# samholt/NeuralLaplaceControl

Hardware: AMD Instinct MI355X
Metric: MPPI planning steps/sec (16384 samples, H=40) (higher is better)
Workload: dtype f64

## Files before the change

### neurallaplacecontrol_amd/csrc/abi_ctx.hip

```cpp
#include "nlc_host.h"

using namespace nlc;
using namespace nlc::host;

namespace nlc {
namespace host {

thread_local std::string g_create_error;

bool gru_use_coop(const nlc_ctx* c, int64_t n_windows) {
  if (c->opt.gru_coop >= 0) return c->opt.gru_coop != 0;
  if (c->g == 128) return true;
  return n_windows <= (c->g == 32 ? 8192 : 50000);
}

void prof_flush(nlc_ctx* c) {
  for (auto& p : c->prof) {
    for (auto& ev : p.pending) {
      hipEventSynchronize(ev.second);
      float ms = 0.f;
      hipEventElapsedTime(&ms, ev.first, ev.second);
      p.total_ms += ms;
      c->event_pool.push_back(ev.first);
      c->event_pool.push_back(ev.second);
// ... 74 lines not shown
    return NLC_OK;
  } catch (...) {
    g_create_error = "exception in nlc_create";
    return NLC_ERR_STATE;
  }
}

extern "C" void nlc_destroy(nlc_ctx* c) {
  if (!c) return;
  hipSetDevice(c->device);
  hipStreamSynchronize(c->stream);
  nlc_comm_destroy(c);
  prof_flush(c);
  if (c->arena.base) hipFree(c->arena.base);
  if (c->dbg_scratch) hipFree(c->dbg_scratch);
  if (c->rnn_base) hipFree(c->rnn_base);
  if (c->node_base) hipFree(c->node_base);
  if (c->slot_dev) hipFree(c->slot_dev);
  if (c->eidx_dev) hipFree(c->eidx_dev);
  if (c->lin_tab) hipFree(c->lin_tab);
  for (int i = 0; i < 2; ++i)
    if (c->U[i]) hipFree(c->U[i]);
  if (c->b1fold) hipFree(c->b1fold);
  if (c->cp_lin) hipFree(c->cp_lin);
  if (c->b1fold_fwd) hipFree(c->b1fold_fwd);
  if (c->small) hipFree(c->small);
  if (c->pinned) hipHostFree(c->pinned);
  c->dh.destroy();
  c->side.destroy();
  for (hipEvent_t e : c->event_pool) hipEventDestroy(e);
// ... 67 lines not shown
  } else if (n == "fused_roll_cap") {
    if (value < 0) return fail(c, NLC_ERR_BAD_ARG, "fused_roll_cap must be >= 0 (0 = auto)");
    c->opt.fused.roll_cap = (int)value;
  } else if (n == "fused_chain_first_tiles") {
    if (value < -1 || value > 64) return fail(c, NLC_ERR_BAD_ARG, "fused_chain_first_tiles must be in -1..64 (-1 = auto)");
    c->opt.fused.chain_first_tiles = (int)value;
  } else if (n == "fused_partner_tiles") {
    if (value < -2 || value > 64) return fail(c, NLC_ERR_BAD_ARG, "fused_partner_tiles must be in -2..64 (-2 = auto, -1 = never)");
    c->opt.fused.partner_tiles = (int)value;
  } else if (n == "repfunc_split") {
    if (value != 0 && value != 1) return fail(c, NLC_ERR_BAD_ARG, "repfunc_split must be 0 or 1");
    c->opt.repfunc_split = (int)value;
  } else if (n == "gru_coop") {
    if (value != 0 && value != 1 && value != -1) return fail(c, NLC_ERR_BAD_ARG, "gru_coop must be -1 (auto), 0 or 1");
    c->opt.gru_coop = (int)value;
  } else if (n == "gru_gemm") {
    if (value != 0 && value != 1) return fail(c, NLC_ERR_BAD_ARG, "gru_gemm must be 0 (FP64 MFMA) or 1 (int8-sliced)");
    c->opt.gru_gemm = (int)value;
    if (c->has_model) c->gru.use_i8 = (c->gru.i8_stream != nullptr && value == 1) ? 1 : 0;
  } else if (n == "dbg_gap_us") {
    if (value < 0 || value > 1.0e5) return fail(c, NLC_ERR_BAD_ARG, "dbg_gap_us must be in 0 .. 1e5");
    c->opt.dbg_gap_us = value;
  } else if (n == "dbg_l2_mb") {
    if (value < 0 || value > 4096) return fail(c, NLC_ERR_BAD_ARG, "dbg_l2_mb must be in 0 .. 4096");
    c->opt.dbg_l2_mb = value;
  } else if (n == "fused_max_samples") {
    if (value < 0) return fail(c, NLC_ERR_BAD_ARG, "fused_max_samples must be >= 0");
    c->opt.fused_max_samples = (int64_t)value;
  } else {
    return fail(c, NLC_ERR_BAD_ARG, "unknown option: " + n);
// ... 5 lines not shown
  if (!c) return NLC_ERR_BAD_ARG;
  if (!name || !out) return fail(c, NLC_ERR_BAD_ARG, "NULL stat name / out");
  const std::string n(name);
  if (n == "rollout_body") *out = (double)c->last_body;
  else if (n == "fused_timeouts") *out = (double)c->fused.timeouts;
  else if (n == "fused_fallbacks") *out = (double)c->fused.fallbacks;
  else if (n == "fused_lost") *out = c->fused.lost ? 1.0 : 0.0;
  else if (n == "last_giveup_command") *out = (double)c->fused.last_giveup_command;
  else if (n == "commands") *out = (double)c->commands;
  else if (n == "comm_world") *out = c->comm ? (double)c->comm_world : 0.0;
  else if (n == "comm_rank") *out = c->comm ? (double)c->comm_rank : -1.0;
  else if (n == "fused_blocks_per_cu") *out = (double)c->fused.blocks_per_cu;
  else if (n == "fused_spin_limit") *out = (double)c->opt.fused_spin_limit;
  else if (n == "model_nt3") *out = c->has_model ? (double)c->net.nt3 : 0.0;
  else if (n == "gru_gemm") *out = (c->has_model && c->gru.use_i8) ? 1.0 : 0.0;
  else if (n == "gru_i8_launches") *out = (double)nlc::gru_i8_launch_count();
  else return fail(c, NLC_ERR_BAD_ARG, "unknown stat: " + n);
  return NLC_OK;
}

extern "C" int nlc_synchronize(nlc_ctx* c) {
  if (!c) return NLC_ERR_BAD_ARG;
  NLC_HIP(c, hipStreamSynchronize(c->stream));
  return NLC_OK;
}

extern "C" int nlc_device_info(nlc_ctx* c, char* name, int name_len, int* cus, int* mhz, double* gib) {
  if (!c) return NLC_ERR_BAD_ARG;
  if (name && name_len > 0) {
    std::snprintf(name, name_len, "%s (%s)", c->prop.name, c->prop.gcnArchName);
// ... 34 lines not shown
```

### neurallaplacecontrol_amd/csrc/abi_model.hip

```cpp
#include "nlc_host.h"

using namespace nlc;
using namespace nlc::host;

namespace {
int64_t blob_size(const nlc_model_desc* d) {
  const int64_t g = d->h / 2, S = d->ilt.terms, P = d->d + 2, h = d->h;
  return 3 * g * d->nin + 3 * g * g + 6 * g + 3 * g * g + 3 * g * g + 6 * g + 2 * g + 2 + h * (2 * S + P) + h +
         h * h + h + 2 * d->d * S * h + 2 * d->d * S;
}
}

extern "C" int64_t nlc_model_blob_size(const nlc_model_desc* d) { return d ? blob_size(d) : -1; }

extern "C" int nlc_set_model(nlc_ctx* c, const nlc_model_desc* d, const double* w, int64_t n) {
  if (!c) return NLC_ERR_BAD_ARG;
  NLC_GUARD_BEGIN
  if (!d || !w) return fail(c, NLC_ERR_BAD_ARG, "NULL desc or weights");
  if (int r = check_ilt(c, &d->ilt)) return r;
  if (d->h != 64 && d->h != 128 && d->h != 256)
    return fail(c, NLC_ERR_UNSUPPORTED, "hidden_units must be 64, 128 or 256 (the kernels are instantiated for these widths)");
  if (d->d < 1 || d->d > 6) return fail(c, NLC_ERR_UNSUPPORTED, "state_dim must be in 1..6");
  if (d->nin < 1 || d->nin > NLC_MAX_NIN) return fail(c, NLC_ERR_UNSUPPORTED, "GRU input dim must be in 1..3");
  const bool linear_algo = d->ilt.algo == NLC_ILT_FIXED_TALBOT || d->ilt.algo == NLC_ILT_STEHFEST;
// ... 55 lines not shown
  const size_t o_W1p = ar.push(pack_A(W1p.data(), 8, 8, rowsh));
  const size_t o_b1 = ar.push(std::vector<double>(b1, b1 + h));
  const size_t o_W2 = ar.push(pack_A(W2, h, h, rowsh));
  const size_t o_b2 = ar.push(std::vector<double>(b2, b2 + h));
  const int nt3 = nl_pick_nt3(ilt_tiles_needed(dd, S));
  if (nt3 < 0) return fail(c, NLC_ERR_UNSUPPORTED, "2*d*S too large for the fused kernel (max 25 output tiles)");
  const IltSlots slots = make_ilt_slots(dd, S, nt3);
  c->slot_elems = slots.elems;
  const int n_even_groups = slots.n_even_groups;
  std::vector<double> b3p((size_t)nt3 * 16, 0.0);
  for (size_t i = 0; i < slots.rowmap3.size(); ++i)
    if (slots.rowmap3[i] >= 0) b3p[i] = b3[slots.rowmap3[i]];
  const size_t o_W3 = ar.push(pack_A(W3, h, h, slots.rowmap3));
  const size_t o_b3 = ar.push(b3p);
  const size_t o_Cp = ar.push(slots.Cp);

  double* base = nullptr;
  NLC_HIP(c, hipMalloc((void**)&base, ar.host.size() * sizeof(double)));
  hipError_t e = hipMemcpy(base, ar.host.data(), ar.host.size() * sizeof(double), hipMemcpyHostToDevice);
  if (e != hipSuccess) {
    hipFree(base);
    return fail(c, NLC_ERR_HIP, std::string("weight upload: ") + hipGetErrorString(e));
  }
  {
    std::vector<int> slot((size_t)nt3 * 8, -1);
    for (size_t i = 0; i < slot.size(); ++i)
      if (slots.elems[i].first >= 0) slot[i] = slots.elems[i].first * S + slots.elems[i].second;
    if (c->slot_dev) hipFree(c->slot_dev);
    c->slot_dev = nullptr;
    NLC_HIP(c, hipMalloc((void**)&c->slot_dev, slot.size() * sizeof(int)));
// ... 49 lines not shown
  N.W1s = base + o_W1s;
  N.b1 = base + o_b1;
  N.W2p = base + o_W2;
  N.b2 = base + o_b2;
  N.W3p = base + o_W3;
  N.b3p = base + o_b3;
  N.Cp = base + o_Cp;
  for (int i = 0; i < NLC_MAX_D; ++i) {
    N.state_mean[i] = i < dd ? d->state_mean[i] : 0.0;
    N.state_std[i] = i < dd ? d->state_std[i] : 1.0;
  }
  N.alpha = d->ilt.alpha;
  N.log_tol = std::log(d->ilt.tol);
  N.scale = d->ilt.scale;
  N.time_div = d->time_div;
  c->has_model = true;
  c->fwd_tn = -1.0;
  c->has_mppi = false;
  return NLC_OK;
  NLC_GUARD_END(c)
}

extern "C" int nlc_gru_encode(nlc_ctx* c, const double* window, int64_t N, int B, double* out) {
  if (!c) return NLC_ERR_BAD_ARG;
  NLC_GUARD_BEGIN
  if (!c->has_model) return fail(c, NLC_ERR_STATE, "nlc_set_model has not been called");
  if (N < 0 || B < 1) return fail(c, NLC_ERR_BAD_SHAPE, "bad N or B");
  if (N == 0) return NLC_OK;
  if (!window || !out) return fail(c, NLC_ERR_BAD_ARG, "NULL device pointer");
  NLC_HIP(c, hipSetDevice(c->device));
// ... 215 lines not shown
```

### neurallaplacecontrol_amd/csrc/abi_planner.hip

```cpp
#include "nlc_host.h"

using namespace nlc;
using namespace nlc::host;

extern "C" int nlc_mppi_configure(nlc_ctx* c, const nlc_mppi_desc* d) {
  if (!c) return NLC_ERR_BAD_ARG;
  NLC_GUARD_BEGIN
  if (!d) return fail(c, NLC_ERR_BAD_ARG, "NULL desc");
  if (d->K < 1 || d->T < 1 || d->K_global < d->K || d->k_offset < 0 || d->k_offset + d->K > d->K_global)
    return fail(c, NLC_ERR_BAD_SHAPE, "bad K / K_global / k_offset / T");
  if (d->nu < 1 || d->nu > NLC_MAX_NU) return fail(c, NLC_ERR_UNSUPPORTED, "nu must be 1 or 2");
  if (d->d < 1 || (d->d > NLC_MAX_D && d->dynamics != NLC_DYN_EXTERNAL)) return fail(c, NLC_ERR_BAD_SHAPE, "bad nx");
  if (d->B < 1) return fail(c, NLC_ERR_BAD_SHAPE, "action_buffer needs at least one row");
  if (!(d->lambda_ > 0.0) || d->u_scale == 0.0) return fail(c, NLC_ERR_BAD_ARG, "lambda_ must be > 0, u_scale != 0");
  if (d->u_per_command < 1 || d->u_per_command > d->T) return fail(c, NLC_ERR_BAD_ARG, "bad u_per_command");
  if (d->E < 0 || d->E > 65535) return fail(c, NLC_ERR_BAD_ARG, "episodes E must be in [0, 65535]");
  const int E = d->E < 1 ? 1 : d->E;
  if ((double)E * (double)d->K * d->T * d->nu > 2.0e9)
    return fail(c, NLC_ERR_BAD_SHAPE, "E*K*T*nu exceeds the planner's index range");
  const bool env_free = d->cost_external &&
                        (d->dynamics == NLC_DYN_NL || d->dynamics == NLC_DYN_DTRNN || d->dynamics == NLC_DYN_NODE) &&
                        d->env == -1;
  if (!env_free && (d->env < 0 || d->env > NLC_ENV_CARTPOLE_NOTRIG)) return fail(c, NLC_ERR_UNSUPPORTED, "unknown env id");
  static const int env_d[4] = {5, 3, 6, 4}, env_nu[4] = {1, 1, 2, 1};
// ... 64 lines not shown
        for (int lane = 0; lane < 64; ++lane) {
          const auto el = c->slot_elems[(size_t)4 * g + (lane >> 4)];
          if (el.first != (lane & 15)) continue;
          cp[(size_t)g * 64 + lane] = tab[2 * S + el.second] / c->tn;
          cp[(size_t)(ng + g) * 64 + lane] = -tab[3 * S + el.second] / c->tn;
        }
      if (c->opt.test_lin_coeff_scale != 1.0) {
        size_t at = 0;
        for (size_t i = 0; i < cp.size(); ++i)
          if (std::fabs(cp[i]) > std::fabs(cp[at])) at = i;
        cp[at] *= c->opt.test_lin_coeff_scale;
      }
      if (int rc = hold_doubles(c, c->cp_lin, cp.size(), cp.data())) return rc;
    }
  }
  c->has_mppi = true;
  c->dh.reset();
  c->wait.reset();
  c->fused.new_problem();
  return NLC_OK;
  NLC_GUARD_END(c)
}

namespace nlc {
namespace host {
bool linear_on_rollout_kernels(const nlc_ctx* c) {
  return c->has_model && (c->md.ilt.algo == NLC_ILT_FIXED_TALBOT || c->md.ilt.algo == NLC_ILT_STEHFEST) &&
         (c->md.h == 64 || c->md.h == 128 || c->md.h == 256) && c->opt.linear_fused != 0;
}

// ... 522 lines not shown
```

### neurallaplacecontrol_amd/csrc/abi_planner_nl.hip

```cpp
#include "nlc_host.h"

using namespace nlc;
using namespace nlc::host;

namespace {

__global__ void dbg_spin_kernel(unsigned long long ticks_100mhz) {
  const unsigned long long t0 = __builtin_amdgcn_s_memrealtime();
  while (__builtin_amdgcn_s_memrealtime() - t0 < ticks_100mhz) __builtin_amdgcn_s_sleep(8);
}
__global__ void dbg_touch_kernel(const double* __restrict__ p, size_t n, double* __restrict__ sink) {
  double acc = 0.0;
  for (size_t i = (size_t)blockIdx.x * blockDim.x + threadIdx.x; i < n; i += (size_t)gridDim.x * blockDim.x) acc += p[i];
  if (acc == 12345.678) *sink = acc;
}
int dbg_between(nlc_ctx* c) {
  if (c->opt.dbg_gap_us > 0.0) hipLaunchKernelGGL(dbg_spin_kernel, dim3(1), dim3(64), 0, c->stream, (unsigned long long)(c->opt.dbg_gap_us * 100.0));
  if (c->opt.dbg_l2_mb > 0.0) {
    const size_t bytes = (size_t)(c->opt.dbg_l2_mb * 1048576.0);
    const size_t n = bytes / 8 + 1;
    if (c->dbg_scratch_n < n) {
      if (int rc = hold_doubles(c, c->dbg_scratch, n, nullptr, &c->dbg_scratch_n)) return rc;
      NLC_HIP(c, hipMemsetAsync(c->dbg_scratch, 0, n * sizeof(double), c->stream));
    }
// ... 314 lines not shown
  }
  c->fused.sync_clean_ws = nullptr;
  c->fused.sync_dirty = true;
  c->fused.last.fused = true;
  c->last_body = 3;
  f.p = p;
  if (fc.inline_weights) f.w = make_weight_args(c, buf);
  {
    ProfScope ps(c, "nl_plan_fused_kernel");
    NLC_HIP(c, launch_nl_plan_fused(f, c->g, s.grid, s.built, c->stream));
  }
  *weights_done = fc.inline_weights != 0;
  return NLC_OK;
}

int rollout_nl_two_launch(nlc_ctx* c, RolloutCall& call, GruArgs& g, RolloutArgs& r, int variant) {
  const nlc_mppi_desc& d = c->pd;
  const int64_t KE = call.KE;
  if (int rc2 = nlc::host::launch_shift_perturb(c, call)) return rc2;
  const plan::Chunks ck = plan::horizon_chunks((variant != 2 && KE > 8192 && d.E == 1) ? c->opt.horizon_chunks : 1, d.T);
  const int C = ck.C, Tc = ck.Tc;
  if (C == 1) {
    g.t0 = 0;
    g.Tc = d.T;
    g.N = KE * d.T;
    {
      ProfScope ps(c, "gru_encode_kernel");
      NLC_HIP(c, launch_gru_encode(g, c->g, c->stream, gru_use_coop(c, g.N)));
    }
    if (c->opt.dbg_gap_us > 0.0 || c->opt.dbg_l2_mb > 0.0)
      if (int rc3 = dbg_between(c)) return rc3;
    r.t_begin = 0;
    r.t_end = d.T;
    ProfScope ps(c, "nl_rollout_kernel");
    NLC_HIP(c, launch_nl_rollout(r, c->stream, variant));
  } else {
    if (int rc = gru_encode_chunks(c, g, KE, C, Tc, false, 0u)) return rc;
    for (int ch = 0; ch < C; ++ch) {
      r.t_begin = ch * Tc;
      r.t_end = (r.t_begin + Tc <= d.T) ? r.t_begin + Tc : d.T;
      if (r.t_begin >= r.t_end) break;
      NLC_HIP(c, hipStreamWaitEvent(c->stream, c->side.ev_gru[ch], 0));
      ProfScope ps(c, "nl_rollout_kernel");
      NLC_HIP(c, launch_nl_rollout(r, c->stream, 1));
    }
  }
  return NLC_OK;
}

}

int nlc::host::rollout_nl(nlc_ctx* c, RolloutCall& call) {
  const nlc_mppi_desc& d = c->pd;
  const nlc_mppi_buffers* buf = call.buf;
  const WsLayout& w = call.w;
  double* ws = call.ws;
  const int64_t KE = call.KE;
  const bool replay = call.replay;
  const bool lin_direct = linear_on_rollout_kernels(c);
  double* pa = ws + w.pa;
  GruArgs g = c->gru;
  g.mode = 1;
  g.perturbed = buf->perturbed;
  g.abuf = call.abuf_dev;
// ... 9 lines not shown
  r.Kep = sc.Kep;
  r.net = c->net;
  r.net.b1 = c->b1fold;
  r.B = d.B;
  r.pa = pa;
  r.tn = c->tn;
  r.xcarry = ws + w.xcarry;
  r.ccarry = ws + w.ccarry;
  if (lin_direct) {
    if (!c->cp_lin) return fail(c, NLC_ERR_STATE, "linear-algorithm coefficient tables missing (nlc_mppi_configure)");
    const size_t ng = (size_t)2 * c->net.nt3 * 64;
    r.net.Cp = c->cp_lin;
    r.net.Cp2 = c->cp_lin + ng;
    r.net.lin = 1;
  }
  if (c->md.ilt.algo != NLC_ILT_FOURIER && !lin_direct) return rollout_nl_staged(c, call, sc, g, r, pa);
  int variant = c->opt.rollout_variant;
  const int h_ = c->md.h;
  const bool fused_ok = (h_ == 64 || h_ == 128 || h_ == 256) && 2 * c->g == h_ && c->net.nt3 <= 21 &&
                        KE * d.T * 16 < (int64_t)1 << 31 && !lin_direct;
  if (variant == 3 && !fused_ok) return fail(c, NLC_ERR_UNSUPPORTED, "fused planner body: model shape not instantiated");
  const int bpc_hi = h_ == 256 ? 2 : 4, bpc_lo = h_ == 256 ? 2 : 3;
  if (fused_ok && (c->fused.blocks_per_cu < 0 || c->fused.occ_h != h_)) {
    int bpc = 0;
    NLC_HIP(c, fused_max_resident_blocks(h_, bpc_hi, &bpc));
    c->fused.blocks_per_cu = bpc;
    NLC_HIP(c, fused_max_resident_blocks(h_, bpc_lo, &bpc));
    c->fused.blocks_per_cu3 = bpc;
    c->fused.occ_h = h_;
  }
  if (variant == 3 && c->fused.blocks_per_cu < 2)
    return fail(c, NLC_ERR_UNSUPPORTED, "fused planner body: fewer than two workgroups of the kernel fit a CU");
  const bool sharded = d.K_global > d.K;
  const bool fold_inside = (c->opt.fused_inline & 1) && d.E == 1 && !d.cost_external;
  if (variant == 0 && fused_ok && c->fused.blocks_per_cu >= 2 && KE <= c->opt.fused_max_samples && (!sharded || fold_inside)) variant = 3;
  if (variant == 3 && (replay || c->fused.lost)) variant = 2;
  const bool in_body = variant == 3 || variant == 2 || (variant == 0 && KE <= 8192);
  if (in_body) cost_in_body(r, d);
  if (variant == 3) {
    bool weights_done = false;
    if (int rc2 = rollout_nl_fused(c, call, g, r, &weights_done)) return rc2;
    if (weights_done) return NLC_OK;
  } else {
    if (int rc2 = rollout_nl_two_launch(c, call, g, r, variant)) return rc2;
    c->last_body = (variant == 2 || (variant == 0 && KE <= 8192)) ? 2 : 1;
  }
  return finish_rollout_costs(c, buf, in_body);
}
```

### neurallaplacecontrol_amd/csrc/kernels_gru.hip

```cpp
#include "nlc_device.h"
#include "nlc_gru_tile.h"
#include "nlc_kernels.h"

namespace nlc {

template <int G>
__global__ __launch_bounds__(256, G <= 64 ? 2 : 1) void gru_encode_kernel(const GruArgs a) {
  constexpr int KS = G / 4;
  const int lane = threadIdx.x & 63, wave = threadIdx.x >> 6;
  const int q = lane >> 4, c = lane & 15;
  const int64_t w = ((int64_t)blockIdx.x * 4 + wave) * 16 + c;
  const bool valid = w < a.N;
  const int64_t wc = valid ? w : a.N - 1;
  int64_t kk = 0;
  int tt = 0;
  if (a.mode == 1) {
    kk = wc / a.Tc;
    tt = a.t0 + (int)(wc - kk * a.Tc);
  }
  __shared__ double Hs[4][2][KS * 64];
  const double o = gru_encode_tile<G>(a, lane, wc, kk, tt, Hs[wave][0], Hs[wave][1]);
  if (valid && q < 2) {
    const int64_t wo = (a.mode == 1) ? kk * a.T + tt : w;
    a.out[wo * 2 + q] = o;
// ... 38 lines not shown
      hipLaunchKernelGGL(gru_encode_coop_kernel<32>, cgrid, dim3(256), lds_pad_bytes, s, a);
    } else if (g == 128) {
      hipLaunchKernelGGL(gru_encode_coop_kernel<128>, cgrid, dim3(256), lds_pad_bytes, s, a);
    } else {
      return hipErrorInvalidValue;
    }
    return hipGetLastError();
  }
  const unsigned grid = (unsigned)((a.N + 63) / 64);
  if (g == 64) {
    hipLaunchKernelGGL((gru_encode_kernel<64>), dim3(grid), dim3(256), 0, s, a);
  } else if (g == 32) {
    hipLaunchKernelGGL((gru_encode_kernel<32>), dim3(grid), dim3(256), 0, s, a);
  } else if (g == 128) {
    hipLaunchKernelGGL((gru_encode_kernel<128>), dim3(grid), dim3(256), 0, s, a);
  } else {
    return hipErrorInvalidValue;
  }
  return hipGetLastError();
}

template <int G, int WPB>
__global__ __launch_bounds__(64 * WPB, G <= 64 ? 2 : 1) void rnn_encode_kernel(const RnnArgs a) {
  constexpr int GT = G / 16;
  constexpr int KS = G / 4;
  const int lane = threadIdx.x & 63, wave = threadIdx.x >> 6;
  const int q = lane >> 4, c = lane & 15;
  const int64_t w = ((int64_t)blockIdx.x * WPB + wave) * 16 + c;
  const bool valid = w < a.N;
  const int64_t wc = valid ? w : a.N - 1;
// ... 77 lines not shown
```

### neurallaplacecontrol_amd/csrc/nlc_gru_tile.h

```cpp
#pragma once
#include "nlc_device.h"
#include "nlc_kernels.h"

namespace nlc {

template <int KS>
__device__ __forceinline__ void chunk_gemm(v4d& c0, v4d& c1, v4d& c2, const double* __restrict__ wc, int lane,
                                           const double* __restrict__ hb) {
  double a_cur[3], a_nxt[3];
  gptr p = opaque(wc);
#pragma unroll
  for (int g = 0; g < 3; ++g) a_cur[g] = p[g * 64 + lane];
  double b_cur = hb[lane], b_nxt = 0.0;
#pragma unroll
  for (int ks = 0; ks < KS; ++ks) {
    if (ks + 1 < KS) {
      p = opaque(p + 3 * 64);
#pragma unroll
      for (int g = 0; g < 3; ++g) a_nxt[g] = p[g * 64 + lane];
      b_nxt = hb[(ks + 1) * 64 + lane];
    }
    c0 = mfma(a_cur[0], b_cur, c0);
    c1 = mfma(a_cur[1], b_cur, c1);
    c2 = mfma(a_cur[2], b_cur, c2);
// ... 63 lines not shown
    const v2d r2 = half ? ar.zw : ar.xy, z2 = half ? az.zw : az.xy, in2 = half ? ain.zw : ain.xy;
    const v2d hn2 = half ? ahn.zw : ahn.xy, ho2 = half ? hold.zw : hold.xy;
    v2d rg, zg;
    sigmoid_pair2(r2, z2, &rg, &zg);
    const v2d ng = tanh2(fma2(rg, hn2, in2));
    const v2d hv = fma2(zg, ho2 - ng, ng);
    if (half) {
      hnew.zw = hv;
    } else {
      hnew.xy = hv;
    }
  }
  return hnew;
}

template <int G>
__device__ __forceinline__ double gru_encode_tile(const GruArgs& a, int lane, int64_t wc, int64_t kk, int tt,
                                                  double* __restrict__ H0, double* __restrict__ H1) {
  constexpr int GT = G / 16;
  constexpr int KS = G / 4;
  const int q = lane >> 4;
  double in_mean = 0.0, in_std = 1.0;
  if (q < a.nin) {
    in_mean = a.mean[q];
    in_std = a.std[q];
  }
  const int ab_off = (a.mode == 1) ? (int)(kk / a.Kep) * a.B : 0;
#pragma unroll
  for (int ks = 0; ks < KS; ++ks) {
    H0[ks * 64 + lane] = 0.0;
    H1[ks * 64 + lane] = 0.0;
  }
  v4d hn[GT];
  bool bad_input = false;

  for (int s = 0; s < a.B; ++s) {
    const int j_win = a.B - 1 - s;
    double xin = 0.0;
    if (q < a.nin) {
      double raw;
      if (a.mode == 0) {
        raw = a.window[(wc * a.B + j_win) * a.nin + q];
      } else {
        const int i = tt + j_win;
        if (q < a.nact)
          raw = (i < a.B - 1) ? a.abuf[(ab_off + 1 + i) * a.nact + q]
                              : a.u_scale * a.perturbed[(kk * a.T + (i - (a.B - 1))) * a.nact + q];
        else
          raw = (double)(a.B - 1 - j_win);
      }
      xin = (raw - in_mean) / in_std;
// ... 21 lines not shown
    for (int j = 0; j < GT; ++j) {
      v4d ar = load_bias_tile(a.brz1, j, q);
      v4d az = load_bias_tile(a.brz1, GT + j, q);
      v4d ain = load_bias_tile(a.bin1, j, q);
      v4d ahn = load_bias_tile(a.bhn1, j, q);
      chunk_gemm<KS>(ar, az, ain, a.Wih1p + (size_t)j * KS * 3 * 64, lane, H0);
      if (s > 0) chunk_gemm<KS>(ar, az, ahn, a.Whh1p + (size_t)j * KS * 3 * 64, lane, H1);
      const v4d hold = {H1[(4 * j + 0) * 64 + lane], H1[(4 * j + 1) * 64 + lane], H1[(4 * j + 2) * 64 + lane],
                        H1[(4 * j + 3) * 64 + lane]};
      hn[j] = gru_gates(ar, az, ain, ahn, hold);
    }
#pragma unroll
    for (int j = 0; j < GT; ++j)
#pragma unroll
      for (int r = 0; r < 4; ++r) H1[(4 * j + r) * 64 + lane] = hn[j][r];
  }
  v4d o[1];
  o[0] = splat(0.0);
  gemm_acc<1, KS>(o, a.Wop, lane, [&](int ks) { return H1[ks * 64 + lane]; });
  return nan_if_bad_window(bad_input, o[0][0] + a.bo[q < 2 ? q : 0]);
}

struct XDirect {
  __device__ __forceinline__ void prepare(const GruArgs&, int, int, int64_t, int, bool) {}
  __device__ __forceinline__ double raw(const GruArgs& a, int64_t wc, int64_t kk, int tt, int j_win, int q, int c,
                                        int ab_off) const {
    if (a.mode == 0) return a.window[(wc * a.B + j_win) * a.nin + q];
    const int i = tt + j_win;
    if (q < a.nact)
      return (i < a.B - 1) ? a.abuf[(ab_off + 1 + i) * a.nact + q]
// ... 99 lines not shown
```

### neurallaplacecontrol_amd/csrc/nlc_host.h

```cpp
#pragma once
#include <dlfcn.h>
#include <hip/hip_runtime.h>

#include <time.h>

#include <cmath>
#include <cstdio>
#include <cstdlib>
#include <cstring>
#include <stdexcept>
#include <string>
#include <vector>

#include "nlc_kernels.h"
#include "nlc_pack.h"
#include "nlc_plan.h"

namespace nlc {
int nl_pick_nt3(int need);

namespace host {

struct ProfEntry {
  std::string name;
  double total_ms = 0.0;
  int64_t launches = 0;
  std::vector<std::pair<hipEvent_t, hipEvent_t>> pending;
};
// ... 3 lines not shown
  size_t n = 0;
  std::vector<double> host;
  size_t push(const std::vector<double>& v) {
    const size_t off = (host.size() + 63) / 64 * 64;
    host.resize(off);
    host.insert(host.end(), v.begin(), v.end());
    return off;
  }
};


struct PlannerOptions {
  int rollout_variant = 0;
  int repfunc_split = 1;
  int gru_coop = -1;
  int gru_gemm = 0;
  int horizon_chunks = 1;
  int dehoog_gru_chunks = 0;
  int dehoog_gru_lds_pad = 49152;
  int dehoog_chain = -1;
  int dehoog_chain_phases = 3;
  int dehoog_streams = 0;
  int linear_fused = 1;
  int host_spin = 1;
  double host_spin_margin_us = 150.0;
  nlc::plan::FusedKnobs fused;
  int64_t fused_max_samples = 4096;
  int fused_inline = 3;
  int64_t fused_spin_limit = 1 << 18;
  int fused_keep_sync = 0;
// ... 34 lines not shown
  float ms[3][2] = {{1e30f, 1e30f}, {1e30f, 1e30f}, {1e30f, 1e30f}};
  hipEvent_t ev[2] = {nullptr, nullptr};
  void reset() {
    n = 0;
    choice = pending = -1;
    for (auto& v : ms) v[0] = v[1] = 1e30f;
  }
  void destroy() {
    for (hipEvent_t& e : ev) {
      if (e) hipEventDestroy(e);
      e = nullptr;
    }
  }
};

struct HostWait {
  unsigned long long seq = 0;
  double hist_us[8] = {0};
  int hist_n = 0, hist_at = 0;
  double nap_margin_us = 0.0;
  void reset() {
    hist_n = hist_at = 0;
    nap_margin_us = 0.0;
  }
};

struct SideStreams {
  hipStream_t gru_stream = nullptr;
  std::vector<hipEvent_t> ev_gru;
  std::vector<hipStream_t> aux_streams;
// ... 61 lines not shown
  int64_t commands = 0;
  int last_body = 0;

  bool profiling = false;
  std::vector<nlc::host::ProfEntry> prof;
  std::vector<hipEvent_t> event_pool;

  double* pinned = nullptr;
  size_t pinned_n = 0;
  nlc::plan::PinLayout pin{};
  nlc::host::PlannerOptions opt;
  nlc::host::FusedState fused;
  nlc::host::DehoogCalib dh;
  nlc::host::HostWait wait;
  nlc::host::SideStreams side;
  double* dbg_scratch = nullptr;
  size_t dbg_scratch_n = 0;
  void* comm = nullptr;
  int comm_world = 0, comm_rank = 0;
  double* comm_gather = nullptr;
  size_t comm_gather_n = 0;
};

namespace nlc {
namespace host {

extern thread_local std::string g_create_error;

inline int fail(nlc_ctx* c, int code, const std::string& msg) {
  if (c) c->err = msg;
// ... 157 lines not shown
struct RolloutCall {
  const nlc_mppi_buffers* buf;
  PerturbArgs p;
  WsLayout w;
  double* ws;
  double* state_dev;
  double* abuf_dev;
  int64_t KE;
  int state_per_sample, rng;
  bool inline_inputs;
  bool replay;
};
int launch_shift_perturb(nlc_ctx* c, RolloutCall& call);
SampleCostArgs sample_cost_args(const nlc_ctx* c, const RolloutCall& call);
int rollout_nl(nlc_ctx* c, RolloutCall& call);

}
}
```

### neurallaplacecontrol_amd/csrc/nlc_kernels.h

```cpp
#pragma once
#include <hip/hip_runtime.h>
#include <stdint.h>

#include <climits>
#include <type_traits>

#include "../../include/nlc.h"
#include "nlc_ilt_tile.h"

namespace nlc {

struct IltArgs {
  const double* theta;
  const double* phi;
  const double* t;
  double* x;
  int64_t N;
  int d, S;
  double alpha, log_tol, scale;
  const double* fre;
  const double* fim;
  double t_div;
  int t_stride;
  int rpp, iters;
// ... 87 lines not shown
  const double* Wih1p;
  const double* Whh1p;
  const double* Wop;
  const double* bhn0;
  const double* brz1;
  const double* bin1;
  const double* bhn1;
  double bo[2];
  double* out;
  int use_i8;
  const signed char* i8_stream;
};
hipError_t launch_gru_encode(const GruArgs& a, int g, hipStream_t s, bool coop = false, unsigned lds_pad_bytes = 0);
hipError_t launch_gru_encode_i8(const GruArgs& a, hipStream_t s);
unsigned long long gru_i8_launch_count();

struct SampleCostArgs {
  int64_t K;
  int64_t Kep;
  int T;
  int nu;
  int env;
  int state_per_sample;
  const double* state0;
  const double* perturbed;
  const double* noise;
  const double* U;
  double sigma_inv[NLC_MAX_NU * NLC_MAX_NU];
  double lambda_;
  double u_scale;
// ... 410 lines not shown
```

### neurallaplacecontrol_amd/planners/mppi_delay.py

```python

import ctypes as C

import torch
from torch.distributions.multivariate_normal import MultivariateNormal

from .. import _lib, _recognise
from ..envs import EnvCost, NLDynamics, OracleDynamics
from ..sharding import (all_ranks_agree, check_same_on_all_ranks, gather_partials, merge_partials_torch, replicate_from_rank0, shard_partials_torch,
                        shard_range, share_bytes_from_rank0, slice_noise)


def _backend_is_rccl(group):
    import torch.distributed as dist

    return str(dist.get_backend(group)).lower() == "nccl"


def _per_dim(v, nu, name):
    t = torch.as_tensor(v, dtype=torch.float64).detach().cpu().reshape(-1)
    if t.numel() == 1:
        t = t.expand(nu)
    if t.numel() != nu:
        raise ValueError(f"{name} must be a scalar or have nu={nu} entries")
    return [float(x) for x in t]
# ... 398 lines not shown

    @property
    def rollout_body(self):
        if self.torch_path:
            return "callables-torch" if self._cost_total is not None else None
        return self._BODIES.get(int(self.ctx.get_stat("rollout_body")))

    @property
    def fused_timeouts(self):
        return 0 if self.torch_path else int(self.ctx.get_stat("fused_timeouts"))

    @property
    def fused_fallbacks(self):
        return 0 if self.torch_path else int(self.ctx.get_stat("fused_fallbacks"))

    noise = property(lambda self: self._out(self._noise))
    perturbed_action = property(lambda self: self._out(self._perturbed))
    states = property(lambda self: self._out(self._states))
    actions = property(lambda self: self._out(self._actions))
    cost_total = property(lambda self: self._out(self._cost_total))
    cost_total_non_zero = property(lambda self: self._out(self._cost_nz))
    omega = property(lambda self: self._out(self._omega))

    def command(self, state, action_buffer):
        if not torch.is_tensor(state):
            state = torch.tensor(state)
        self._state_in = state
        if self.torch_path:
            return self._torch_command(state, action_buffer)
        st = state.detach().to("cpu", torch.float64).contiguous()
# ... 207 lines not shown
```

Baseline: 244.2.

## Reuse precomputed GRU encoder prefixes for windows with saturated actions

Adds a prefix table built once at planner setup. It holds the GRU hidden states for every pattern of up to four leading action-buffer entries that sit exactly at the upper or lower action bound. Each call, a new index kernel classifies every encoder window by how many leading inputs match a bound bit-for-bit and buckets the windows into per-length lists. A new encoder kernel then seeds each tile from the table and skips those recurrent steps. This targets redundant GRU steps when many sampled actions are clamped. In exchange it adds an extra classification pass with atomics, a compaction step, and padded tiles per list. It only applies to the two-launch, non-cooperative FP64 path with one action dimension and bounds.

```diff
diff --git a/neurallaplacecontrol_amd/csrc/abi_ctx.hip b/neurallaplacecontrol_amd/csrc/abi_ctx.hip
--- a/neurallaplacecontrol_amd/csrc/abi_ctx.hip
+++ b/neurallaplacecontrol_amd/csrc/abi_ctx.hip
@@ -112,6 +112,7 @@
   prof_flush(c);
   if (c->arena.base) hipFree(c->arena.base);
   if (c->dbg_scratch) hipFree(c->dbg_scratch);
+  if (c->prefix.lists) hipFree(c->prefix.lists);
   if (c->rnn_base) hipFree(c->rnn_base);
   if (c->node_base) hipFree(c->node_base);
   if (c->slot_dev) hipFree(c->slot_dev);
@@ -209,6 +210,9 @@
   } else if (n == "gru_coop") {
     if (value != 0 && value != 1 && value != -1) return fail(c, NLC_ERR_BAD_ARG, "gru_coop must be -1 (auto), 0 or 1");
     c->opt.gru_coop = (int)value;
+  } else if (n == "gru_prefix") {
+    if (value != 0 && value != 1 && value != -1) return fail(c, NLC_ERR_BAD_ARG, "gru_prefix must be -1 (auto), 0 or 1");
+    c->opt.gru_prefix = (int)value;
   } else if (n == "gru_gemm") {
     if (value != 0 && value != 1) return fail(c, NLC_ERR_BAD_ARG, "gru_gemm must be 0 (FP64 MFMA) or 1 (int8-sliced)");
     c->opt.gru_gemm = (int)value;
@@ -244,6 +248,16 @@
   else if (n == "fused_spin_limit") *out = (double)c->opt.fused_spin_limit;
   else if (n == "model_nt3") *out = c->has_model ? (double)c->net.nt3 : 0.0;
   else if (n == "gru_gemm") *out = (c->has_model && c->gru.use_i8) ? 1.0 : 0.0;
+  else if (n == "gru_prefix") *out = c->prefix.last_used ? 1.0 : 0.0;
+  else if (n.rfind("gru_prefix_windows_l", 0) == 0 && n.size() == 21 && n[20] >= '0' && n[20] <= '4') {
+    *out = 0.0;
+    if (c->prefix.last_used && c->prefix.lists) {
+      unsigned cnt[nlc::prefix::kLists] = {0};
+      NLC_HIP(c, hipStreamSynchronize(c->stream));
+      NLC_HIP(c, hipMemcpy(cnt, c->prefix.lists, sizeof(cnt), hipMemcpyDeviceToHost));
+      *out = (double)cnt[n[20] - '0'];
+    }
+  } else if (n == "latents_offset") *out = (c->has_mppi && c->pd.dynamics == NLC_DYN_NL) ? (double)ws_layout(c).pa : -1.0;
   else if (n == "gru_i8_launches") *out = (double)nlc::gru_i8_launch_count();
   else return fail(c, NLC_ERR_BAD_ARG, "unknown stat: " + n);
   return NLC_OK;
diff --git a/neurallaplacecontrol_amd/csrc/abi_model.hip b/neurallaplacecontrol_amd/csrc/abi_model.hip
--- a/neurallaplacecontrol_amd/csrc/abi_model.hip
+++ b/neurallaplacecontrol_amd/csrc/abi_model.hip
@@ -93,6 +93,7 @@
   const size_t o_W3 = ar.push(pack_A(W3, h, h, slots.rowmap3));
   const size_t o_b3 = ar.push(b3p);
   const size_t o_Cp = ar.push(slots.Cp);
+  const size_t o_prefix = ar.push(std::vector<double>(gru_prefix_arena_doubles(g), 0.0));
 
   double* base = nullptr;
   NLC_HIP(c, hipMalloc((void**)&base, ar.host.size() * sizeof(double)));
@@ -172,6 +173,8 @@
   N.log_tol = std::log(d->ilt.tol);
   N.scale = d->ilt.scale;
   N.time_div = d->time_div;
+  c->prefix.arena_off = o_prefix;
+  c->prefix.why_not = "gru_prefix: planner not configured";
   c->has_model = true;
   c->fwd_tn = -1.0;
   c->has_mppi = false;
diff --git a/neurallaplacecontrol_amd/csrc/abi_planner.hip b/neurallaplacecontrol_amd/csrc/abi_planner.hip
--- a/neurallaplacecontrol_amd/csrc/abi_planner.hip
+++ b/neurallaplacecontrol_amd/csrc/abi_planner.hip
@@ -102,6 +102,9 @@
       if (int rc = hold_doubles(c, c->cp_lin, cp.size(), cp.data())) return rc;
     }
   }
+  c->prefix.last_used = false;
+  if (d->dynamics == NLC_DYN_NL)
+    if (int rc = gru_prefix_configure(c)) return rc;
   c->has_mppi = true;
   c->dh.reset();
   c->wait.reset();
diff --git a/neurallaplacecontrol_amd/csrc/abi_planner_nl.hip b/neurallaplacecontrol_amd/csrc/abi_planner_nl.hip
--- a/neurallaplacecontrol_amd/csrc/abi_planner_nl.hip
+++ b/neurallaplacecontrol_amd/csrc/abi_planner_nl.hip
@@ -352,9 +352,46 @@
   return NLC_OK;
 }
 
+int gru_prefix_begin(nlc_ctx* c, RolloutCall& call, const GruArgs& g, int64_t N, int chunks, bool* use, GruPrefixArgs* px) {
+  *use = false;
+  if (c->opt.gru_prefix == 0) return NLC_OK;
+  GruPrefixState& ps = c->prefix;
+  const char* why = ps.why_not;
+  if (!why && ps.last_B != g.B) why = "gru_prefix: the table was built for another action-buffer length";
+  if (!why && chunks != 1) why = "gru_prefix: not with the encoder in horizon chunks (horizon_chunks)";
+  if (!why && gru_use_coop(c, N)) why = "gru_prefix: this launch takes the cooperative encoder (gru_coop)";
+  if (!why && g.use_i8) why = "gru_prefix: the FP64 encoder only (gru_gemm is 1)";
+  if (!why) why = prefix::out_of_scope(g.nact, g.nin, 1, g.B, N, true);
+  if (why) return c->opt.gru_prefix == 1 ? fail(c, NLC_ERR_UNSUPPORTED, why) : NLC_OK;
+  const int64_t stride = (N + 63) / 64 * 64;
+  const size_t need = 64 + (size_t)prefix::kLists * (size_t)stride / 2;
+  if (need > ps.lists_n) {
+    NLC_HIP(c, hipStreamSynchronize(c->stream));
+    if (int rc = hold_doubles(c, ps.lists, need, nullptr, &ps.lists_n)) return rc;
+  }
+  double* base = c->arena.base + ps.arena_off;
+  px->table = base;
+  px->out_tab = base + (size_t)prefix::kEntries * 2 * c->g;
+  px->counts = reinterpret_cast<unsigned*>(ps.lists);
+  px->lists = reinterpret_cast<unsigned*>(ps.lists + 64);
+  px->list_stride = stride;
+  px->img_max = ps.img_max;
+  px->img_min = ps.img_min;
+  call.p.zero_words = px->counts;
+  call.p.n_zero_words = 16;
+  *use = true;
+  return NLC_OK;
+}
+
 int rollout_nl_two_launch(nlc_ctx* c, RolloutCall& call, GruArgs& g, RolloutArgs& r, int variant) {
   const nlc_mppi_desc& d = c->pd;
   const int64_t KE = call.KE;
+  bool use_prefix = false;
+  GruPrefixArgs px{};
+  {
+    const int chunks = plan::horizon_chunks((variant != 2 && KE > 8192 && d.E == 1) ? c->opt.horizon_chunks : 1, d.T).C;
+    if (int rc = gru_prefix_begin(c, call, g, KE * d.T, chunks, &use_prefix, &px)) return rc;
+  }
   if (int rc2 = nlc::host::launch_shift_perturb(c, call)) return rc2;
   const plan::Chunks ck = plan::horizon_chunks((variant != 2 && KE > 8192 && d.E == 1) ? c->opt.horizon_chunks : 1, d.T);
   const int C = ck.C, Tc = ck.Tc;
@@ -362,7 +399,15 @@
     g.t0 = 0;
     g.Tc = d.T;
     g.N = KE * d.T;
-    {
+    if (use_prefix) {
+      {
+        ProfScope ps(c, "gru_prefix_index_kernel");
+        NLC_HIP(c, launch_gru_prefix_index(g, px, c->stream));
+      }
+      ProfScope ps(c, "gru_encode_kernel");
+      NLC_HIP(c, launch_gru_encode_prefix(g, px, c->g, c->stream));
+      c->prefix.last_used = true;
+    } else {
       ProfScope ps(c, "gru_encode_kernel");
       NLC_HIP(c, launch_gru_encode(g, c->g, c->stream, gru_use_coop(c, g.N)));
     }
@@ -386,6 +431,44 @@
   return NLC_OK;
 }
 
+}
+
+int nlc::host::gru_prefix_configure(nlc_ctx* c) {
+  const nlc_mppi_desc& d = c->pd;
+  GruPrefixState& ps = c->prefix;
+  ps.last_B = d.B;
+  ps.last_used = false;
+  const double img[2] = {prefix::bound_image(d.u_max[0], d.u_scale), prefix::bound_image(d.u_min[0], d.u_scale)};
+  bool finite = true;
+  for (double v : img) finite = finite && std::isfinite((d.u_scale * v - c->gru.mean[0]) / c->gru.std[0]);
+  ps.why_not = prefix::out_of_scope(d.nu, c->md.nin, d.has_bounds, d.B, 0, finite);
+  if (ps.why_not) return NLC_OK;
+  ps.img_max = prefix::bits_of(img[0]);
+  ps.img_min = prefix::bits_of(img[1]);
+  std::vector<double> syn((size_t)16 * d.B, 0.0);
+  for (int col = 0; col < 16; ++col)
+    for (int s = 0; s < prefix::cap(d.B); ++s) syn[(size_t)col * d.B + (d.B - 1 - s)] = img[(col >> s) & 1];
+  double* base = c->arena.base + ps.arena_off;
+  GruPrefixArgs px{};
+  px.table = base;
+  px.out_tab = base + (size_t)prefix::kEntries * 2 * c->g;
+  double* syn_dev = px.out_tab + 64;
+  NLC_HIP(c, hipMemcpy(syn_dev, syn.data(), syn.size() * sizeof(double), hipMemcpyHostToDevice));
+  GruArgs a = c->gru;
+  a.mode = 1;
+  a.perturbed = syn_dev;
+  a.abuf = syn_dev;
+  a.u_scale = d.u_scale;
+  a.T = a.Tc = d.B;
+  a.t0 = 0;
+  a.Kep = 16;
+  a.N = 16;
+  a.B = d.B;
+  a.nact = 1;
+  a.out = nullptr;
+  NLC_HIP(c, launch_gru_prefix_table(a, px, c->g, c->stream));
+  NLC_HIP(c, hipStreamSynchronize(c->stream));
+  return NLC_OK;
 }
 
 int nlc::host::rollout_nl(nlc_ctx* c, RolloutCall& call) {
@@ -425,7 +508,12 @@
     r.net.Cp2 = c->cp_lin + ng;
     r.net.lin = 1;
   }
-  if (c->md.ilt.algo != NLC_ILT_FOURIER && !lin_direct) return rollout_nl_staged(c, call, sc, g, r, pa);
+  c->prefix.last_used = false;
+  const char* prefix_two_launch_only = "gru_prefix: the encoder launch of the two-launch body only (rollout_variant 1 / 2)";
+  if (c->md.ilt.algo != NLC_ILT_FOURIER && !lin_direct) {
+    if (c->opt.gru_prefix == 1) return fail(c, NLC_ERR_UNSUPPORTED, prefix_two_launch_only);
+    return rollout_nl_staged(c, call, sc, g, r, pa);
+  }
   int variant = c->opt.rollout_variant;
   const int h_ = c->md.h;
   const bool fused_ok = (h_ == 64 || h_ == 128 || h_ == 256) && 2 * c->g == h_ && c->net.nt3 <= 21 &&
@@ -449,6 +537,7 @@
   const bool in_body = variant == 3 || variant == 2 || (variant == 0 && KE <= 8192);
   if (in_body) cost_in_body(r, d);
   if (variant == 3) {
+    if (c->opt.gru_prefix == 1) return fail(c, NLC_ERR_UNSUPPORTED, prefix_two_launch_only);
     bool weights_done = false;
     if (int rc2 = rollout_nl_fused(c, call, g, r, &weights_done)) return rc2;
     if (weights_done) return NLC_OK;
diff --git a/neurallaplacecontrol_amd/csrc/kernels_gru.hip b/neurallaplacecontrol_amd/csrc/kernels_gru.hip
--- a/neurallaplacecontrol_amd/csrc/kernels_gru.hip
+++ b/neurallaplacecontrol_amd/csrc/kernels_gru.hip
@@ -1,4 +1,5 @@
 #include "nlc_device.h"
+#include "nlc_gru_prefix.h"
 #include "nlc_gru_tile.h"
 #include "nlc_kernels.h"
 
@@ -76,6 +77,148 @@
     hipLaunchKernelGGL((gru_encode_kernel<32>), dim3(grid), dim3(256), 0, s, a);
   } else if (g == 128) {
     hipLaunchKernelGGL((gru_encode_kernel<128>), dim3(grid), dim3(256), 0, s, a);
+  } else {
+    return hipErrorInvalidValue;
+  }
+  return hipGetLastError();
+}
+
+
+template <int G>
+__global__ __launch_bounds__(64) void gru_prefix_table_kernel(const GruArgs a, const GruPrefixArgs px) {
+  constexpr int KS = G / 4;
+  const int lane = threadIdx.x & 63;
+  const int q = lane >> 4, c = lane & 15;
+  __shared__ double Hs[2][KS * 64];
+  for (int i = lane; i < 2 * G; i += 64) px.table[i] = 0.0;
+  const int steps = prefix::cap(a.B);
+  const double o = gru_encode_tile<G, true>(a, lane, c, c, a.B - 1, Hs[0], Hs[1], 0, steps, px.table);
+  if (steps == a.B && q < 2 && c < (1 << steps)) px.out_tab[prefix::entry_index(steps, c) * 2 + q] = o;
+}
+
+constexpr int kIndexPerThread = 8;
+__global__ __launch_bounds__(256) void gru_prefix_index_kernel(const GruArgs a, const GruPrefixArgs px) {
+  __shared__ unsigned cnt[8], base[8];
+  const int lane = threadIdx.x & 63;
+  const int nl = prefix::n_lists(a.B);
+  if (threadIdx.x < 8) cnt[threadIdx.x] = 0u;
+  __syncthreads();
+  const int64_t w0 = (int64_t)blockIdx.x * (256 * kIndexPerThread) + threadIdx.x;
+  unsigned cls[kIndexPerThread];
+#pragma unroll
+  for (int it = 0; it < kIndexPerThread; ++it) {
+    const int64_t w = w0 + it * 256;
+    int len = 7, pattern = 0;
+    if (w < a.N) {
+      const int64_t kk = w / a.Tc;
+      const int tt = a.t0 + (int)(w - kk * a.Tc);
+      const prefix::Class c = prefix::classify(a.perturbed + kk * a.T, tt, a.B, px.img_max, px.img_min);
+      len = c.len;
+      pattern = c.pattern;
+      if (len == a.B) {
+        const double* o = px.out_tab + prefix::entry_index(len, pattern) * 2;
+        a.out[(kk * a.T + tt) * 2 + 0] = o[0];
+        a.out[(kk * a.T + tt) * 2 + 1] = o[1];
+      }
+    }
+    cls[it] = (unsigned)len | ((unsigned)pattern << 3);
+    for (int l = 0; l <= prefix::kMaxLen; ++l) {
+      const unsigned long long m = __ballot(len == l);
+      if (m != 0ull && lane == __ffsll((long long)m) - 1) atomicAdd(&cnt[l], (unsigned)__popcll(m));
+    }
+  }
+  __syncthreads();
+  if (threadIdx.x <= prefix::kMaxLen) {
+    const unsigned n = cnt[threadIdx.x];
+    base[threadIdx.x] = n ? atomicAdd(px.counts + threadIdx.x, n) : 0u;
+    cnt[threadIdx.x] = 0u;
+  }
+  __syncthreads();
+#pragma unroll
+  for (int it = 0; it < kIndexPerThread; ++it) {
+    const int64_t w = w0 + it * 256;
+    const int len = (int)(cls[it] & 7u);
+    for (int l = 0; l < nl; ++l) {
+      const unsigned long long m = __ballot(len == l);
+      if (m == 0ull) continue;
+      const int leader = __ffsll((long long)m) - 1;
+      unsigned b = 0u;
+      if (lane == leader) b = atomicAdd(&cnt[l], (unsigned)__popcll(m));
+      b = (unsigned)__shfl((int)b, leader);
+      if (len == l) {
+        const unsigned pos = base[l] + b + (unsigned)__popcll(m & ((1ull << lane) - 1ull));
+        if ((int64_t)pos < px.list_stride) px.lists[(int64_t)l * px.list_stride + pos] = (unsigned)w | ((cls[it] >> 3) << prefix::kPatternShift);
+      }
+    }
+  }
+}
+
+template <int G>
+__global__ __launch_bounds__(256, G <= 64 ? 2 : 1) void gru_encode_prefix_kernel(const GruArgs a, const GruPrefixArgs px) {
+  constexpr int KS = G / 4;
+  const int lane = threadIdx.x & 63;
+  const int wave = __builtin_amdgcn_readfirstlane(threadIdx.x >> 6);
+  const int q = lane >> 4, c = lane & 15;
+  const int nl = prefix::n_lists(a.B);
+  int64_t tile = (int64_t)blockIdx.x * 4 + wave;
+  int len = 0;
+  unsigned n = 0u;
+  for (; len < nl; ++len) {
+    n = px.counts[len];
+    if ((int64_t)n > px.list_stride) n = (unsigned)px.list_stride;
+    const int64_t nt = ((int64_t)n + 15) / 16;
+    if (tile < nt) break;
+    tile -= nt;
+  }
+  if (len == nl) return;
+  const int64_t idx = tile * 16 + c;
+  const bool valid = idx < (int64_t)n;
+  const unsigned e = px.lists[(int64_t)len * px.list_stride + (valid ? idx : (int64_t)n - 1)];
+  int64_t w = (int64_t)(e & ((1u << prefix::kPatternShift) - 1u));
+  if (w >= a.N) w = a.N - 1;
+  const int64_t kk = w / a.Tc;
+  const int tt = a.t0 + (int)(w - kk * a.Tc);
+  __shared__ double Hs[4][2][KS * 64];
+  if (len > 0) {
+    const int pattern = (int)(e >> prefix::kPatternShift) & ((1 << len) - 1);
+    const double* ent = px.table + (size_t)prefix::entry_index(len, pattern) * 2 * G;
+#pragma unroll
+    for (int ks = 0; ks < KS; ++ks) {
+      Hs[wave][0][ks * 64 + lane] = ent[4 * ks + q];
+      Hs[wave][1][ks * 64 + lane] = ent[G + 4 * ks + q];
+    }
+  }
+  const double o = gru_encode_tile<G, true>(a, lane, w, kk, tt, Hs[wave][0], Hs[wave][1], len);
+  if (valid && q < 2) a.out[(kk * a.T + tt) * 2 + q] = o;
+}
+
+hipError_t launch_gru_prefix_table(const GruArgs& a, const GruPrefixArgs& px, int g, hipStream_t s) {
+  if (g == 64) {
+    hipLaunchKernelGGL(gru_prefix_table_kernel<64>, dim3(1), dim3(64), 0, s, a, px);
+  } else if (g == 32) {
+    hipLaunchKernelGGL(gru_prefix_table_kernel<32>, dim3(1), dim3(64), 0, s, a, px);
+  } else if (g == 128) {
+    hipLaunchKernelGGL(gru_prefix_table_kernel<128>, dim3(1), dim3(64), 0, s, a, px);
+  } else {
+    return hipErrorInvalidValue;
+  }
+  return hipGetLastError();
+}
+hipError_t launch_gru_prefix_index(const GruArgs& a, const GruPrefixArgs& px, hipStream_t s) {
+  if (a.N <= 0) return hipSuccess;
+  const int64_t per_block = 256 * kIndexPerThread;
+  hipLaunchKernelGGL(gru_prefix_index_kernel, dim3((unsigned)((a.N + per_block - 1) / per_block)), dim3(256), 0, s, a, px);
+  return hipGetLastError();
+}
+hipError_t launch_gru_encode_prefix(const GruArgs& a, const GruPrefixArgs& px, int g, hipStream_t s) {
+  if (a.N <= 0) return hipSuccess;
+  const unsigned grid = (unsigned)((prefix::worst_case_tiles(a.N, a.B) + 3) / 4);
+  if (g == 64) {
+    hipLaunchKernelGGL(gru_encode_prefix_kernel<64>, dim3(grid), dim3(256), 0, s, a, px);
+  } else if (g == 32) {
+    hipLaunchKernelGGL(gru_encode_prefix_kernel<32>, dim3(grid), dim3(256), 0, s, a, px);
+  } else if (g == 128) {
+    hipLaunchKernelGGL(gru_encode_prefix_kernel<128>, dim3(grid), dim3(256), 0, s, a, px);
   } else {
     return hipErrorInvalidValue;
   }
diff --git a/neurallaplacecontrol_amd/csrc/nlc_gru_prefix.h b/neurallaplacecontrol_amd/csrc/nlc_gru_prefix.h
--- /dev/null
+++ b/neurallaplacecontrol_amd/csrc/nlc_gru_prefix.h
@@ -0,0 +1,63 @@
+#pragma once
+#include <cstdint>
+
+#if defined(__HIPCC__)
+#define NLC_PREFIX_HD __host__ __device__
+#else
+#define NLC_PREFIX_HD
+#endif
+
+namespace nlc {
+namespace prefix {
+
+constexpr int kMaxLen = 4;
+constexpr int kEntries = (2 << kMaxLen) - 1;
+constexpr int kLists = kMaxLen + 1;
+constexpr int kMaxB = 32;
+constexpr int kPatternShift = 27;
+constexpr int64_t kMaxWindows = (int64_t)1 << kPatternShift;
+
+NLC_PREFIX_HD inline uint64_t bits_of(double x) {
+  uint64_t u;
+  __builtin_memcpy(&u, &x, sizeof(u));
+  return u;
+}
+NLC_PREFIX_HD inline double bound_image(double bound, double u_scale) { return bound / u_scale; }
+NLC_PREFIX_HD inline int cap(int B) { return B < kMaxLen ? B : kMaxLen; }
+NLC_PREFIX_HD inline int n_lists(int B) { return B < kLists ? B : kLists; }
+NLC_PREFIX_HD inline int entry_index(int len, int pattern) { return (1 << len) - 1 + pattern; }
+
+struct Class {
+  int len, pattern;
+};
+NLC_PREFIX_HD inline Class classify(const double* row, int t, int B, uint64_t img_max, uint64_t img_min) {
+  Class c{0, 0};
+  const int L = cap(B);
+  for (int s = 0; s < L; ++s) {
+    const int i = t + B - 1 - s;
+    if (i < B - 1) break;
+    const uint64_t v = bits_of(row[i - (B - 1)]);
+    if (v == img_max) {
+    } else if (v == img_min) {
+      c.pattern |= 1 << s;
+    } else {
+      break;
+    }
+    c.len = s + 1;
+  }
+  return c;
+}
+
+NLC_PREFIX_HD inline int64_t worst_case_tiles(int64_t N, int B) { return N / 16 + n_lists(B); }
+
+inline const char* out_of_scope(int nu, int nin, int has_bounds, int B, int64_t N, bool images_finite) {
+  if (nu != 1 || nin != 1) return "gru_prefix: one action dimension and no time channel only (nu == nin == 1)";
+  if (!has_bounds) return "gru_prefix: the planner has no action bounds";
+  if (B > kMaxB) return "gru_prefix: action buffers of up to 32 rows only";
+  if (N > kMaxWindows) return "gru_prefix: at most 2^27 windows per launch";
+  if (!images_finite) return "gru_prefix: a bound's normalised image is not finite";
+  return nullptr;
+}
+
+}
+}
diff --git a/neurallaplacecontrol_amd/csrc/nlc_gru_tile.h b/neurallaplacecontrol_amd/csrc/nlc_gru_tile.h
--- a/neurallaplacecontrol_amd/csrc/nlc_gru_tile.h
+++ b/neurallaplacecontrol_amd/csrc/nlc_gru_tile.h
@@ -101,9 +101,10 @@
   return hnew;
 }
 
-template <int G>
+template <int G, bool kPrefix = false>
 __device__ __forceinline__ double gru_encode_tile(const GruArgs& a, int lane, int64_t wc, int64_t kk, int tt,
-                                                  double* __restrict__ H0, double* __restrict__ H1) {
+                                                  double* __restrict__ H0, double* __restrict__ H1, int s0 = 0,
+                                                  int s_end = -1, double* __restrict__ dump = nullptr) {
   constexpr int GT = G / 16;
   constexpr int KS = G / 4;
   const int q = lane >> 4;
@@ -113,15 +114,17 @@
     in_std = a.std[q];
   }
   const int ab_off = (a.mode == 1) ? (int)(kk / a.Kep) * a.B : 0;
-#pragma unroll
-  for (int ks = 0; ks < KS; ++ks) {
-    H0[ks * 64 + lane] = 0.0;
-    H1[ks * 64 + lane] = 0.0;
+  if (!kPrefix || s0 == 0) {
+#pragma unroll
+    for (int ks = 0; ks < KS; ++ks) {
+      H0[ks * 64 + lane] = 0.0;
+      H1[ks * 64 + lane] = 0.0;
+    }
   }
   v4d hn[GT];
   bool bad_input = false;
 
-  for (int s = 0; s < a.B; ++s) {
+  for (int s = kPrefix ? s0 : 0; s < ((kPrefix && s_end >= 0) ? s_end : a.B); ++s) {
     const int j_win = a.B - 1 - s;
     double xin = 0.0;
     if (q < a.nin) {
@@ -173,6 +176,14 @@
     for (int j = 0; j < GT; ++j)
 #pragma unroll
       for (int r = 0; r < 4; ++r) H1[(4 * j + r) * 64 + lane] = hn[j][r];
+    if (kPrefix && dump != nullptr && (lane & 15) < (2 << s)) {
+      double* e = dump + (size_t)((2 << s) - 1 + (lane & 15)) * 2 * G;
+#pragma unroll
+      for (int ks = 0; ks < KS; ++ks) {
+        e[4 * ks + q] = H0[ks * 64 + lane];
+        e[G + 4 * ks + q] = H1[ks * 64 + lane];
+      }
+    }
   }
   v4d o[1];
   o[0] = splat(0.0);
diff --git a/neurallaplacecontrol_amd/csrc/nlc_host.h b/neurallaplacecontrol_amd/csrc/nlc_host.h
--- a/neurallaplacecontrol_amd/csrc/nlc_host.h
+++ b/neurallaplacecontrol_amd/csrc/nlc_host.h
@@ -12,6 +12,7 @@
 #include <string>
 #include <vector>
 
+#include "nlc_gru_prefix.h"
 #include "nlc_kernels.h"
 #include "nlc_pack.h"
 #include "nlc_plan.h"
@@ -45,6 +46,7 @@
   int rollout_variant = 0;
   int repfunc_split = 1;
   int gru_coop = -1;
+  int gru_prefix = -1;
   int gru_gemm = 0;
   int horizon_chunks = 1;
   int dehoog_gru_chunks = 0;
@@ -109,6 +111,16 @@
   }
 };
 
+struct GruPrefixState {
+  size_t arena_off = 0;
+  const char* why_not = "gru_prefix: planner not configured";
+  unsigned long long img_max = 0, img_min = 0;
+  double* lists = nullptr;
+  size_t lists_n = 0;
+  bool last_used = false;
+  int last_B = 0;
+};
+
 struct HostWait {
   unsigned long long seq = 0;
   double hist_us[8] = {0};
@@ -200,6 +212,7 @@
   nlc::host::DehoogCalib dh;
   nlc::host::HostWait wait;
   nlc::host::SideStreams side;
+  nlc::host::GruPrefixState prefix;
   double* dbg_scratch = nullptr;
   size_t dbg_scratch_n = 0;
   void* comm = nullptr;
@@ -387,6 +400,10 @@
 int launch_shift_perturb(nlc_ctx* c, RolloutCall& call);
 SampleCostArgs sample_cost_args(const nlc_ctx* c, const RolloutCall& call);
 int rollout_nl(nlc_ctx* c, RolloutCall& call);
-
-}
-}
+int gru_prefix_configure(nlc_ctx* c);
+inline size_t gru_prefix_arena_doubles(int g) {
+  return (size_t)nlc::prefix::kEntries * 2 * g + 64 + (size_t)16 * nlc::prefix::kMaxB;
+}
+
+}
+}
diff --git a/neurallaplacecontrol_amd/csrc/nlc_kernels.h b/neurallaplacecontrol_amd/csrc/nlc_kernels.h
--- a/neurallaplacecontrol_amd/csrc/nlc_kernels.h
+++ b/neurallaplacecontrol_amd/csrc/nlc_kernels.h
@@ -125,6 +125,17 @@
 hipError_t launch_gru_encode(const GruArgs& a, int g, hipStream_t s, bool coop = false, unsigned lds_pad_bytes = 0);
 hipError_t launch_gru_encode_i8(const GruArgs& a, hipStream_t s);
 unsigned long long gru_i8_launch_count();
+struct GruPrefixArgs {
+  double* table;
+  double* out_tab;
+  unsigned* lists;
+  unsigned* counts;
+  int64_t list_stride;
+  unsigned long long img_max, img_min;
+};
+hipError_t launch_gru_prefix_table(const GruArgs& a, const GruPrefixArgs& px, int g, hipStream_t s);
+hipError_t launch_gru_prefix_index(const GruArgs& a, const GruPrefixArgs& px, hipStream_t s);
+hipError_t launch_gru_encode_prefix(const GruArgs& a, const GruPrefixArgs& px, int g, hipStream_t s);
 
 struct SampleCostArgs {
   int64_t K;
diff --git a/neurallaplacecontrol_amd/planners/mppi_delay.py b/neurallaplacecontrol_amd/planners/mppi_delay.py
--- a/neurallaplacecontrol_amd/planners/mppi_delay.py
+++ b/neurallaplacecontrol_amd/planners/mppi_delay.py
@@ -436,6 +436,20 @@
     def fused_fallbacks(self):
         return 0 if self.torch_path else int(self.ctx.get_stat("fused_fallbacks"))
 
+    @property
+    def gru_prefix(self):
+        if self.torch_path or self.ctx is None or not int(self.ctx.get_stat("gru_prefix")):
+            return False, [0] * 5
+        return True, [int(self.ctx.get_stat(f"gru_prefix_windows_l{i}")) for i in range(5)]
+
+    @property
+    def gru_latents(self):
+        off = -1 if self.torch_path or self._buf is None else int(self.ctx.get_stat("latents_offset"))
+        if off < 0:
+            return None
+        n = self.K_local * self.T * 2 * getattr(self, "E", 1)
+        return self._ws[off:off + n].view(self._lead(self.K_local, self.T, 2))
+
     noise = property(lambda self: self._out(self._noise))
     perturbed_action = property(lambda self: self._out(self._perturbed))
     states = property(lambda self: self._out(self._states))
```

After: 260.8, median of 6. 1.07x the previous value.
